# RobotLocomotion/pytorch-dense-correspondence

Measured on AMD Instinct MI355X. Metric: training images/sec, 640x480 D=3 ResNet34-8s, higher is better.
Workload: dtype f32 (f16x3 products)

## Files before the change

include/dcn_hip.h:

```cpp
#ifndef DCN_HIP_H
#define DCN_HIP_H

#include <stddef.h>
#include <stdint.h>

#ifdef __cplusplus
extern "C" {
#endif

#define DCN_OK 0
#define DCN_E_INVALID (-1)
#define DCN_E_LAUNCH (-2)
#define DCN_E_UNSUPPORTED (-3)

const char* dcn_version(void);

void dcn_reload_env(void);

void dcn_release_pooled_buffers(void);


enum { DCN_LIST_MATCH = 0, DCN_LIST_MASKED = 1, DCN_LIST_BACKGROUND = 2, DCN_LIST_BLIND = 3, DCN_NUM_LISTS = 4 };

enum {
// ... 76 lines not shown
int dcn_plan_bn_info(const dcn_plan* plan, int j, char* name, int name_cap, int64_t* channels);

int dcn_plan_fused_bn_backward(const dcn_plan* plan);

int dcn_plan_num_activation_slots(const dcn_plan* plan);
size_t dcn_plan_activation_absmax_offset(const dcn_plan* plan);

int dcn_plan_num_grad_buckets(const dcn_plan* plan);
int dcn_plan_grad_bucket_first_param(const dcn_plan* plan, int k);
int dcn_plan_stream_wait_grad_bucket(dcn_plan* plan, int k, void* stream);

size_t dcn_plan_saved_bytes(const dcn_plan* plan);
size_t dcn_plan_workspace_bytes(const dcn_plan* plan);
double dcn_plan_forward_flops(const dcn_plan* plan);

int dcn_backbone_forward(dcn_plan* plan, const float* image, const float* const* params,
                         float* const* bn_running, float momentum, float eps, int training, int normalize,
                         float* descriptors, void* saved, void* workspace, void* stream);

int dcn_backbone_forward_pair(dcn_plan* plan, const float* image_a, const float* image_b, const float* const* params,
                              float* const* bn_running, float momentum, float eps, int training, int normalize,
                              float* descriptors, void* saved, void* workspace, void* stream);

int dcn_plan_profile_begin(dcn_plan* plan);
int dcn_plan_profile_end(dcn_plan* plan, double ms[2], int64_t launches[2], double flops[2]);
int dcn_plan_profile_end3(dcn_plan* plan, double ms[3], int64_t launches[3], double flops[3]);
enum {
    DCN_PROF_GEMM = 0,
    DCN_PROF_WGRAD = 1,
    DCN_PROF_GEMM_HL = 2,
    DCN_PROF_BN_APPLY = 3,
    DCN_PROF_BN_BWD_REDUCE = 4,
    DCN_PROF_BN_BWD_APPLY = 5,
    DCN_PROF_BN_FINALIZE = 6,
    DCN_PROF_RESAMPLE = 7,
    DCN_PROF_OTHER = 8,
    DCN_PROF_NCAT = 9
};
int dcn_plan_profile_end_all(dcn_plan* plan, double ms[DCN_PROF_NCAT], int64_t launches[DCN_PROF_NCAT],
                             double work[DCN_PROF_NCAT]);

int dcn_backbone_backward(dcn_plan* plan, const float* grad_descriptors, const float* const* params,
                          const void* saved, void* workspace, float* const* grads, int normalize, void* stream);
int dcn_backbone_backward_pair(dcn_plan* plan, const float* grad_a, const float* grad_b, const float* const* params,
                               const void* saved, void* workspace, float* const* grads, int normalize, void* stream);


typedef struct dcn_conv_desc {
    int32_t n, hin, win, cin;
    int32_t hout, wout, cout;
    int32_t kh, kw, stride, pad, dil;
    int32_t ldc;
    int32_t group_rows;
} dcn_conv_desc;

int dcn_conv_forward(const dcn_conv_desc* c, const float* in, const float* w, const float* bias, float* out,
                     float* bn_partial, void* workspace, void* stream);
size_t dcn_conv_gemm_workspace(const dcn_conv_desc* c, int dgrad);
int dcn_conv_num_mtiles(const dcn_conv_desc* c);
int dcn_conv_dgrad(const dcn_conv_desc* c, const float* dout, const float* wt, const float* add, float* din,
                   void* workspace, void* stream);
int dcn_conv_wgrad(const dcn_conv_desc* c, const float* in, const float* dout, float* dw, void* slabs, void* stream);
size_t dcn_conv_wgrad_workspace(const dcn_conv_desc* c);
int dcn_transpose_weight(const float* w, float* wt, int cout, int taps, int cin, int ldn, void* stream);

int dcn_f16_kpad(int k);
int dcn_split_rows_f16(const float* w, void* hi, void* lo, int64_t rows, int k, float scale, void* stream);
int dcn_conv_num_mtiles_f16(const dcn_conv_desc* c);
size_t dcn_conv_gemm_workspace_f16(const dcn_conv_desc* c, int dgrad);
int dcn_conv_forward_f16(const dcn_conv_desc* c, const float* in, const float* in_absmax, const void* w_hi, const void* w_lo,
                         float w_scale, const float* bias, float* out, float* bn_partial, void* workspace, void* stream);
int dcn_conv_dgrad_f16(const dcn_conv_desc* c, const float* dout, const void* wt_hi, const void* wt_lo, float w_scale,
                       const float* dout_absmax, const float* add, float* din, void* workspace, void* stream);
int dcn_conv_dgrad_bn_num_mtiles_f16(const dcn_conv_desc* c);
int dcn_conv_dgrad_bn_f16(const dcn_conv_desc* c, const float* dout, const void* wt_hi, const void* wt_lo, float w_scale,
                          const float* dout_absmax, const float* add, float* din, const float* bn_x,
                          const unsigned char* relu_mask, const float* bn_stats, float* bn_partial, void* workspace,
                          void* stream);

int dcn_split_weights_checked_f16(int n, const float* const* w, const float* const* row_scale, void* const* hi, void* const* lo,
                                  const int* cout, const int* taps, const int* cin, float scale, int* status, void* stream);

int dcn_conv_hl_eligible(const dcn_conv_desc* c, int dgrad);
int dcn_conv_num_mtiles_hl(const dcn_conv_desc* c);
int dcn_conv_tile_rows_hl(const dcn_conv_desc* c, int dgrad);
size_t dcn_conv_gemm_workspace_hl(const dcn_conv_desc* c, int dgrad);
int dcn_conv_hl_shape_info(const dcn_conv_desc* c, int dgrad, int* info6);
int dcn_split_act_hl32(const float* src, const float* absmax, void* dst, int64_t rows, int channels, void* stream);
int dcn_split_weights_hl32(int n, const float* const* w, void* const* out, const int* cout, const int* taps, const int* cin,
                           const int* ldn, int transposed, float scale, void* stream);
int dcn_conv_forward_hl(const dcn_conv_desc* c, const void* in_hl, const float* in_absmax, const void* w_hl, float w_scale,
                        const float* bias, float* out, float* bn_partial, void* workspace, void* stream);
int dcn_conv_dgrad_hl(const dcn_conv_desc* c, const void* dout_hl, const void* wt_hl, float w_scale, const float* dout_absmax,
                      const float* add, float* din, void* workspace, void* stream);

int dcn_conv_wgrad_hl_eligible(const dcn_conv_desc* c);
int dcn_conv_wgrad_hl_kind(const dcn_conv_desc* c);
size_t dcn_conv_wgrad_workspace_hl(const dcn_conv_desc* c);
int dcn_conv_wgrad_hl(const dcn_conv_desc* c, const void* x_hl, const float* x_absmax, const void* dout_hl,
                      const float* dout_absmax, float* dw, void* slabs, void* stream);

int dcn_split_stem_weights_f16(const float* w4, void* hi, void* lo, int cout, float scale, void* stream);
int dcn_conv_stem_forward_f16(const dcn_conv_desc* c, const float* in, const float* in_absmax, const void* w_hi, const void* w_lo,
                              float w_scale, float* out, float* bn_partial, void* stream);

int dcn_split_weights_f16(int n, const float* const* w, void* const* hi, void* const* lo, const int* cout, const int* taps,
                          const int* cin, const int* ldn, int transposed, float scale, void* stream);

int dcn_split_weights_scaled_f16(int n, const float* const* w, const float* const* row_scale, void* const* hi,
                                 void* const* lo, const int* cout, const int* taps, const int* cin, const int* ldn,
                                 int transposed, float scale, void* stream);
int dcn_conv_forward_fused_f16(const dcn_conv_desc* c, const float* in, const float* in_absmax, const void* w_hi,
                               const void* w_lo, float w_scale, const float* bias, const float* add, int relu, float* out,
                               float* out_absmax, void* workspace, void* stream);

int dcn_split_act_f16(const float* src, void* xs, int64_t n, void* stream);
size_t dcn_grad_blocked_bytes(int m, int ld);
int dcn_split_grad_blocked_f16(const float* dy, int m, int ld, const float* absmax, void* dq, void* stream);
int dcn_conv_wgrad_f16(const dcn_conv_desc* c, const void* xs, int xs_is_fp32, const float* x_absmax, const void* dq,
                       const float* dout_absmax, float* dw, void* slabs, void* stream);
size_t dcn_conv_wgrad_workspace_f16(const dcn_conv_desc* c);

int dcn_bn_forward(const float* x, const float* bn_partial, int mtiles, int c, int64_t rows, const float* gamma,
                   const float* beta, float* running_mean, float* running_var, float momentum, float eps, int training,
                   const float* res, int relu, float* y, unsigned char* relu_mask, float* stats, void* stream);
size_t dcn_bn_backward_workspace(int64_t rows, int c);
int dcn_bn_backward(const float* dy, const unsigned char* relu_mask, const float* x, const float* stats, const float* gamma,
                    int c, int64_t rows, float* dgamma, float* dbeta, float* dx, float* g_out, void* workspace,
                    void* stream);
int dcn_bn_backward_from_partial(const float* dy, const float* bn_partial, int mtiles, const float* x, const float* stats,
                                 const float* gamma, int c, int64_t rows, float* dgamma, float* dbeta, float* dx,
                                 void* workspace, void* stream);
int dcn_maxpool_forward(const float* in, int n, int hin, int win, int c, float* out, unsigned char* argmax, void* stream);
int dcn_maxpool_backward(const float* gout, const unsigned char* argmax, int n, int hin, int win, int c, float* gin,
                         void* stream);

int dcn_upsample_forward(const float* low, int n, int hl, int wl, int ldl, int d, int h, int w, int normalize,
                         float* out, void* stream);
int dcn_upsample_backward(const float* gout, int n, int hl, int wl, int ldl, int d, int h, int w, float* glow,
                          float* tmp, void* stream);
size_t dcn_upsample_backward_tmp_bytes(int n, int hl, int w, int d);

size_t dcn_match_statistics_workspace(int q);
int dcn_match_statistics(const float* res, int64_t hw, int w, int d, const float* queries, const int64_t* gt_idx, int q,
                         const unsigned char* mask, int64_t* best_idx, float* best_dist, int32_t* count, float* dist_sum,
                         float* gt_dist, void* workspace, void* stream);

int dcn_find_best_match(const float* res, int64_t hw, int d, const float* queries, int q, const unsigned char* mask,
                        int64_t* best_idx, float* best_dist, float* norm_diffs, void* workspace, void* stream);
size_t dcn_find_best_match_workspace(int q);

size_t dcn_find_correspondences_workspace(int64_t n);
int dcn_find_correspondences(const uint16_t* depth_a, const uint16_t* depth_b, int h, int w, const float* K,
                             const float* K_inv, const float* pose_a, const float* pose_b_inv, const int64_t* cand_u,
                             const int64_t* cand_v, int64_t n, int64_t* out_ua, int64_t* out_va, float* out_ub,
                             float* out_vb, int64_t* out_count, void* workspace, void* stream);
size_t dcn_mask_nonzero_workspace(int64_t hw);
int dcn_mask_nonzero(const float* mask, int64_t hw, int64_t* list, int64_t* count, void* workspace, void* stream);
int dcn_sample_pixels(const float* rand, int64_t n, int w, int h, const int64_t* list, const int64_t* count, float* u,
                      float* v, void* stream);

int dcn_adam_step(int n, void* const* param, const void* const* grad, void* const* exp_avg, void* const* exp_avg_sq,
                  const int64_t* numel, double lr, double beta1, double beta2, double eps, double weight_decay,
                  int64_t step, void* stream);

#define DCN_AUG_PARAM_WORDS 16
// ... 103 lines not shown
```

pytorch-dense-correspondence_amd/csrc/conv_hl_kernels.hip:

```cpp
#include <algorithm>
#include <atomic>
#include <type_traits>

#include "conv_hlx.h"
#include "conv_shared.h"
#include "dcn_tuning.h"
#include "f16_split.h"

namespace {

using namespace dcnconv;
using namespace dcnsplit;

typedef __attribute__((address_space(3))) void* hl_lds_ptr;

constexpr int kOob = (int)0x80000000;
constexpr int kHlStage = 65536;
template <int MT> struct HlStage {
    static constexpr int kA = MT == 5 ? 320 * 128 : 32768, kStage = kA + 32768;
};
constexpr int HLK = 32;

__device__ __forceinline__ void glds16(__amdgpu_buffer_rsrc_t rs, void* lds_dst, int voffset, int soffset) {
    __builtin_amdgcn_raw_ptr_buffer_load_lds(rs, (hl_lds_ptr)lds_dst, 16, voffset, soffset, 0, 0);
}

__global__ void __launch_bounds__(256)
split_act_hl32_kernel(const float* __restrict__ src, const float* __restrict__ absmax, u32x4* __restrict__ dst, int64_t n8) {
    const float s = absmax ? pow2_scale(*absmax) : 1.f;
    for (int64_t i = (int64_t)blockIdx.x * 256 + threadIdx.x; i < n8; i += (int64_t)gridDim.x * 256) {
        const float4 a = reinterpret_cast<const float4*>(src)[2 * i], b = reinterpret_cast<const float4*>(src)[2 * i + 1];
        h4 ah, al, bh, bl;
        split4(a, s, ah, al);
        split4(b, s, bh, bl);
        const u32x2 h0 = __builtin_bit_cast(u32x2, ah), h1 = __builtin_bit_cast(u32x2, bh);
        const u32x2 l0 = __builtin_bit_cast(u32x2, al), l1 = __builtin_bit_cast(u32x2, bl);
        u32x4* line = dst + (i >> 2) * 8 + (i & 3);
        line[0] = u32x4{h0[0], h0[1], h1[0], h1[1]};
        line[4] = u32x4{l0[0], l0[1], l1[0], l1[1]};
    }
}

template <bool TR, int MT>
__device__ __forceinline__ void gemm_segment_hl(const GemmConv& p, unsigned char* lds, int tile, int k0, int k1, int nk,
                                                float* slot) {
    static_assert(MT == 3 || MT == 4 || MT == 5, "wavefront tiles of 96, 128 or 160 rows");
    constexpr int BM = 64 * MT, GR = 32 * MT;
    constexpr int NA = MT == 4 ? 4 : MT;
    constexpr int kHlStage = HlStage<MT>::kStage, kAB = HlStage<MT>::kA;
    const int tid = threadIdx.x, lane = tid & 63;
    const int wv = __builtin_amdgcn_readfirstlane(tid >> 6);
    const int grp = wv >> 2, wn = wv & 3;
    const int mt = fdiv(tile, p.div_nt), nt = tile - mt * p.ntiles;
    const int m0 = mt * BM, n0 = nt * 256;
    const __amdgpu_buffer_rsrc_t rs_a = __builtin_amdgcn_make_buffer_rsrc(const_cast<float*>(p.src), 0, (int)p.src_bytes, 0x00020000);
    const __amdgpu_buffer_rsrc_t rs_b = __builtin_amdgcn_make_buffer_rsrc(const_cast<_Float16*>(p.wh), 0, (int)p.w_bytes, 0x00020000);

    const int l8 = lane >> 3, ls = lane & 7;
    const int cs4 = p.cs * 4;
    auto a_piece_row = [&](int a) { return MT == 4 ? grp * 128 + (a >> 1) * 64 + (2 * wn + (a & 1)) * 8 : grp * GR + a * 32 + wn * 8; };
    int by[NA], bx[NA], rowoff[NA], voa[NA], vob[2][2];
    unsigned vmask[NA];
    int cur_delta = 0, cur_bit = 0;
#pragma unroll
    for (int a = 0; a < NA; ++a) {
        const int row = a_piece_row(a) + l8;
        const int sl = ls ^ ((row >> 1) & 7);
        const int m = m0 + row;
        const bool ok = m < p.M;
        const int mm = ok ? m : 0;
        const int img = fdiv(mm, p.div_hw), rem = mm - img * p.div_hw.d;
        const int y = fdiv(rem, p.div_w), x = rem - y * p.div_w.d;
        by[a] = ok ? (TR ? y + p.pad : y - p.pad) : -(1 << 28);
        bx[a] = TR ? x + p.pad : x - p.pad;
        rowoff[a] = ok ? (img * p.hs * p.ws + by[a] * p.ws + bx[a]) * cs4 + sl * 16 : 0;
        vmask[a] = 0u;
        if constexpr (MT == 5) {
            const int ntap = p.kh * p.kw;
            for (int tap = 0; tap < ntap; ++tap) {
                const int r = fdiv(tap, p.div_kw), s = tap - r * p.kw;
                const int dy = r * p.dil, dx = s * p.dil;
                bool v;
                if (TR) {
                    const int ny = by[a] - dy, nx = bx[a] - dx;
                    v = ((ny | nx) >= 0) & (ny < p.hs) & (nx < p.ws);
                } else {
// ... 464 lines not shown
    const HlxShape x = hlx_shape(M, cd, K, group_rows, taps, cs);
    const bool x_forced = force == 160 || tune.gemm_hlx_kg > 0 || tune.gemm_hlx_splits > 0;
    if (x.ok && (x_forced || !best.ok || x.cost < 0.97 * best_cost * best.nk)) {
        HlShape gx = best;
        gx.rows = kHlxRows; gx.mtiles = x.mtiles; gx.ntiles = x.ntiles; gx.nk = x.nk;
        gx.sk = false; gx.sk_wgs = 0; gx.sk_units = 0; gx.sk_dp = 0;
        gx.ws_bytes = x.ws_bytes; gx.sk_count_off = x.cnt_off;
        gx.ok = true;
        gx.x = x;
        return gx;
    }
    if (force == 160) best.ok = false;
    return best;
}

bool valid_desc_hl(const dcn_conv_desc* c) {
    return c && c->n > 0 && c->hin > 0 && c->win > 0 && c->cin > 0 && c->hout > 0 && c->wout > 0 && c->cout > 0 && c->kh > 0 &&
           c->kw > 0 && c->stride > 0 && c->dil > 0 && c->pad >= 0 && c->ldc >= c->cout;
}

template <int MT>
void launch_gemm_hl_rows(const GemmConv& p, bool sk, dim3 grid, hipStream_t st) {
    const dim3 block(512);
    if constexpr (MT != 5) {
        if (sk) {
            if (p.transposed) hipLaunchKernelGGL((conv_gemm_hl_kernel<true, true, MT>), grid, block, 0, st, p);
            else hipLaunchKernelGGL((conv_gemm_hl_kernel<false, true, MT>), grid, block, 0, st, p);
            return;
        }
    }
    {
        if (p.transposed) hipLaunchKernelGGL((conv_gemm_hl_kernel<true, false, MT>), grid, block, 0, st, p);
        else hipLaunchKernelGGL((conv_gemm_hl_kernel<false, false, MT>), grid, block, 0, st, p);
    }
}

int launch_gemm_hl(GemmConv& p, int group_rows, void* workspace, hipStream_t st) {
    if (p.relu || p.out_absmax || p.bnb_partial) return DCN_E_UNSUPPORTED;
    p.sshift = 0;
    p.div_hw = make_fastdiv(p.hd * p.wd);
    p.div_w = make_fastdiv(p.wd);
    p.div_cs = make_fastdiv(p.cs);
    p.div_kw = make_fastdiv(p.kw);
    const HlShape g = hl_shape(p.M, p.cd, p.K, group_rows, p.kh * p.kw, p.cs);
    if (!g.ok) return DCN_E_UNSUPPORTED;
    p.hl_setprio = dcn::tuning().hl_setprio;
    if (g.rows == kHlxRows) {
        if (g.x.splits > 1 && !workspace) {
            HlxShape x1 = g.x;
            x1.splits = 1; x1.ws_bytes = 0; x1.cnt_off = 0;
            return launch_gemm_hlx(p, x1, nullptr, st);
        }
        return launch_gemm_hlx(p, g.x, workspace, st);
    }
    const bool sk = g.sk && workspace != nullptr;
    p.mtiles = g.mtiles;
    p.ntiles = g.ntiles;
    p.div_nt = make_fastdiv(g.ntiles);
    p.div_nk = make_fastdiv(g.nk);
    p.sk_units = sk ? g.sk_units : 0;
    p.sk_dp = sk ? g.sk_dp : 0;
    p.sk_partial = sk ? (float*)workspace : nullptr;
    p.sk_count = sk ? (unsigned long long*)((char*)workspace + g.sk_count_off) : nullptr;
    p.sk_bytes = sk ? (unsigned)g.sk_count_off : 0u;
    if (sk) {
        p.sk_id = next_sk_launch_id();
        if (dcn::fill_bytes_async(p.sk_count, 0, (size_t)(g.mtiles * g.ntiles - g.sk_dp) * sizeof(unsigned long long), st) != DCN_OK)
            return DCN_E_LAUNCH;
    }
    const dim3 grid(sk ? g.sk_wgs : g.mtiles * g.ntiles);
    if (g.rows == 192) launch_gemm_hl_rows<3>(p, sk, grid, st);
    else if (g.rows == 320) launch_gemm_hl_rows<5>(p, false, grid, st);
    else launch_gemm_hl_rows<4>(p, sk, grid, st);
    return dcn::check_launch();
}

}

static HlShape hl_shape_of(const dcn_conv_desc* c, int dgrad) {
    if (dgrad) return hl_shape(c->n * c->hin * c->win, c->cin, c->kh * c->kw * c->ldc, 0, c->kh * c->kw, c->ldc);
    return hl_shape(c->n * c->hout * c->wout, c->cout, c->kh * c->kw * c->cin, c->group_rows, c->kh * c->kw, c->cin);
}

static bool hl_supported(const dcn_conv_desc* c, int dgrad) {
    if (!valid_desc_hl(c)) return false;
    if (c->stride != 1 || (c->ldc % 4) != 0) return false;
    const int cs = dgrad ? c->ldc : c->cin, cd = dgrad ? c->cin : c->cout;
    const int64_t M = (int64_t)c->n * (dgrad ? c->hin * c->win : c->hout * c->wout);
    const int64_t K = (int64_t)c->kh * c->kw * cs;
    if ((cs % HLK) != 0 || (dgrad && c->ldc != c->cout) || (cd % 4) != 0 || M >= ((int64_t)1 << 30)) return false;
    if (dgrad && (c->hin != c->hout || c->win != c->wout)) return false;
    const int64_t src_bytes = (int64_t)c->n * (dgrad ? c->hout * c->wout : c->hin * c->win) * cs * 4;
    const int64_t w_bytes = (int64_t)cd * K * 4;
    if (!(src_bytes <= ((int64_t)1 << 31) - 1 && w_bytes <= ((int64_t)1 << 31) - 1)) return false;
    return hl_shape_of(c, dgrad).ok;
}

extern "C" int dcn_conv_hl_eligible(const dcn_conv_desc* c, int dgrad) {
    if (!hl_supported(c, dgrad) || dcn::tuning().gemm_hl == 0) return 0;
    if (dcn::tuning().gemm_hl == 2) return 1;
    const int cs = dgrad ? c->ldc : c->cin, cd = dgrad ? c->cin : c->cout;
    const int64_t M = (int64_t)c->n * (dgrad ? c->hin * c->win : c->hout * c->wout);
    const int64_t K = (int64_t)c->kh * c->kw * cs;
    if (!(cd >= 128 && K >= std::min(512, dcn::tuning().hl_min_k) && M >= 4096)) return 0;
    const HlShape chosen = hl_shape_of(c, dgrad);
    if (chosen.rows == kHlxRows) return (cd >= 256 || cs >= 256 || dcn::tuning().gemm_hlx_narrow != 0) ? 1 : 0;
    if (cd < 256) return 0;
    if (chosen.rows == 320 && chosen.mtiles * chosen.ntiles <= 256 && chosen.mtiles * chosen.ntiles >= 120) return 1;
    const double rounds = (double)dcn::ceil_div64(M, 256) * dcn::ceil_div(cd, 256) / 256.0;
    if (rounds > 1.0 && rounds < 1.5 && K < 4096) return 0;
    if (rounds < 120.0 / 256.0) return 0;
    return 1;
}

extern "C" int dcn_conv_num_mtiles_hl(const dcn_conv_desc* c) {
    if (!valid_desc_hl(c)) return DCN_E_INVALID;
    return hl_shape_of(c, 0).mtiles;
}

extern "C" int dcn_conv_tile_rows_hl(const dcn_conv_desc* c, int dgrad) {
    if (!valid_desc_hl(c)) return DCN_E_INVALID;
    return hl_shape_of(c, dgrad).rows;
}

extern "C" size_t dcn_conv_gemm_workspace_hl(const dcn_conv_desc* c, int dgrad) {
    if (!valid_desc_hl(c)) return 0;
    return hl_shape_of(c, dgrad).ws_bytes;
}

extern "C" int dcn_conv_hl_shape_info(const dcn_conv_desc* c, int dgrad, int* info6) {
    if (!valid_desc_hl(c) || !info6) return DCN_E_INVALID;
    if (!hl_supported(c, dgrad)) return DCN_E_UNSUPPORTED;
    const HlShape g = hl_shape_of(c, dgrad);
    const bool x = g.rows == kHlxRows;
    info6[0] = g.rows; info6[1] = x ? g.x.bn : 256; info6[2] = x ? g.x.kg : 1; info6[3] = x ? g.x.splits : 1;
    info6[4] = g.mtiles; info6[5] = g.ntiles;
    return DCN_OK;
}

extern "C" int dcn_split_act_hl32(const float* src, const float* absmax, void* dst, int64_t rows, int channels, void* stream) {
    if (!src || !dst || rows < 1 || channels < HLK || (channels % HLK) != 0) return DCN_E_INVALID;
    const int64_t n8 = rows * (channels / 8);
    const unsigned blocks = (unsigned)(dcn::ceil_div64(n8, 256) > 8192 ? 8192 : dcn::ceil_div64(n8, 256));
    hipLaunchKernelGGL(split_act_hl32_kernel, dim3(blocks), dim3(256), 0, (hipStream_t)stream, src, absmax, (u32x4*)dst, n8);
    return dcn::check_launch();
}

extern "C" int dcn_conv_forward_hl(const dcn_conv_desc* c, const void* in_hl, const float* in_absmax, const void* w_hl,
                                   float w_scale, const float* bias, float* out, float* bn_partial, void* workspace,
                                   void* stream) {
    if (!in_hl || !w_hl || !out || !(w_scale > 0.f)) return DCN_E_INVALID;
    if (!hl_supported(c, 0)) return DCN_E_UNSUPPORTED;
    GemmConv p;
    p.src = (const float*)in_hl; p.wm = nullptr; p.bias = bias; p.add = nullptr; p.dst = out; p.bn_partial = bn_partial;
    p.out_absmax = nullptr; p.wh = (const _Float16*)w_hl; p.wl = nullptr; p.a_absmax = in_absmax; p.b_inv_scale = 1.f / w_scale;
    p.hs = c->hin; p.ws = c->win; p.cs = c->cin; p.hd = c->hout; p.wd = c->wout; p.cd = c->cout;
    p.kh = c->kh; p.kw = c->kw; p.stride = 1; p.pad = c->pad; p.dil = c->dil; p.ldc = c->ldc;
    p.M = c->n * c->hout * c->wout; p.K = c->kh * c->kw * c->cin; p.kp = p.K; p.transposed = 0; p.relu = 0;
    p.src_bytes = (unsigned)((int64_t)c->n * c->hin * c->win * c->cin * 4);
    p.w_bytes = (unsigned)((int64_t)c->cout * p.K * 4);
    return launch_gemm_hl(p, c->group_rows, workspace, (hipStream_t)stream);
}

extern "C" int dcn_conv_dgrad_hl(const dcn_conv_desc* c, const void* dout_hl, const void* wt_hl, float w_scale,
                                 const float* dout_absmax, const float* add, float* din, void* workspace, void* stream) {
    if (!dout_hl || !wt_hl || !din || !(w_scale > 0.f)) return DCN_E_INVALID;
    if (!hl_supported(c, 1)) return DCN_E_UNSUPPORTED;
    GemmConv p;
    p.src = (const float*)dout_hl; p.wm = nullptr; p.bias = nullptr; p.add = add; p.dst = din; p.bn_partial = nullptr;
    p.out_absmax = nullptr; p.wh = (const _Float16*)wt_hl; p.wl = nullptr; p.a_absmax = dout_absmax; p.b_inv_scale = 1.f / w_scale;
    p.hs = c->hout; p.ws = c->wout; p.cs = c->ldc; p.hd = c->hin; p.wd = c->win; p.cd = c->cin;
    p.kh = c->kh; p.kw = c->kw; p.stride = 1; p.pad = c->pad; p.dil = c->dil; p.ldc = c->cin;
    p.M = c->n * c->hin * c->win; p.K = c->kh * c->kw * c->ldc; p.kp = p.K; p.transposed = 1; p.relu = 0;
    p.src_bytes = (unsigned)((int64_t)c->n * c->hout * c->wout * c->ldc * 4);
    p.w_bytes = (unsigned)((int64_t)c->cin * p.K * 4);
    return launch_gemm_hl(p, 0, workspace, (hipStream_t)stream);
}
```

pytorch-dense-correspondence_amd/csrc/dcn_tuning.h:

```cpp
#pragma once

namespace dcn {

struct Tuning {
    int conv_mode = -1;
    int conv_mode_invalid = 0;
    int backward_overlap = 1;
    int gemm_tile_m = 0;
    int gemm_sk = -1;
    double gemm_sk_min_gain = 20.0;
    int gemm_uni = 1;
    int stem8 = 1;
    int gemm_sk_inline = 1;
    int bn_bwd_fused = 0;
    int defer_residual_add = 1;
    int wgrad_splits = 0;
    int wgrad_tile = 0;
    int wgrad_deep = 4;
    int gemm_hl = 1;
    int hl_min_k = 128;
    int gemm_hl_rows = 0;
    int gemm_hlx = 1;
    int gemm_hlx_kg = 0;
    int gemm_hlx_splits = 0;
    int gemm_hlx_narrow = 1;
    double hlx_cost1 = 1.32, hlx_cost2 = 1.42, hlx_split_cost = 14.0;
    int hl_setprio = 1;
    int hlx_stagger = 1;
    int hlx_counters = 1;
    int wgrad_hl_min_m = 0;
    int wgrad_hl = 1;
    int wgrad_hlr = 1;
    int wgrad_hlr_min_m = 0;
    int wgrad_hlr_pairs = 1;
    int hl_producers = 1;
    int hl_only_mid = 1;
    int stem_pool_fused = 1;
    int bn_reduce_wide = 32;
    int wsplit_overlap = 1;
    int bn_nt = 0;
    int bn_reverse = 0;
    int wgrad_roles = 1;
};

const Tuning& tuning();

}
```

pytorch-dense-correspondence_amd/csrc/dcn_tuning.hip:

```cpp
#include <atomic>
#include <cstdio>
#include <cstdlib>
#include <cstring>
#include <mutex>

#include "dcn_common.h"
#include "dcn_tuning.h"

namespace dcn {
namespace {

Tuning g_tuning;
std::once_flag g_once;
std::mutex g_mu;

void read_env(Tuning& t) {
    t = Tuning();
    if (const char* m = getenv("DCN_CONV_MODE")) {
        if (!strcmp(m, "fp32")) t.conv_mode = DCN_CONV_FP32;
        else if (!strcmp(m, "f16x3")) t.conv_mode = DCN_CONV_F16X3;
        else t.conv_mode_invalid = 1;
    }
    if (const char* e = getenv("DCN_BACKWARD_OVERLAP")) t.backward_overlap = atoi(e) != 0;
    if (const char* e = getenv("DCN_GEMM_TILE_M")) t.gemm_tile_m = atoi(e);
    if (const char* e = getenv("DCN_GEMM_SK")) t.gemm_sk = atoi(e);
    if (const char* e = getenv("DCN_GEMM_SK_MIN_GAIN")) t.gemm_sk_min_gain = atof(e);
    if (const char* e = getenv("DCN_STEM8")) t.stem8 = atoi(e) != 0;
    if (const char* e = getenv("DCN_GEMM_UNI")) t.gemm_uni = atoi(e) != 0;
    if (const char* e = getenv("DCN_GEMM_SK_FIXUP")) t.gemm_sk_inline = strcmp(e, "kernel") != 0;
    if (const char* e = getenv("DCN_BN_BWD_FUSED")) t.bn_bwd_fused = atoi(e) != 0;
    if (const char* e = getenv("DCN_DEFER_RESIDUAL_ADD")) t.defer_residual_add = atoi(e) != 0;
    if (const char* e = getenv("DCN_WGRAD_DEEP")) t.wgrad_deep = atoi(e);
    if (const char* e = getenv("DCN_WGRAD_ROLES")) t.wgrad_roles = atoi(e);
    if (const char* e = getenv("DCN_WGRAD_TILE")) t.wgrad_tile = atoi(e);
    if (const char* e = getenv("DCN_WGRAD_SPLITS")) t.wgrad_splits = atoi(e);
    if (const char* e = getenv("DCN_GEMM_HL")) t.gemm_hl = atoi(e);
    if (const char* e = getenv("DCN_GEMM_HL_ROWS")) t.gemm_hl_rows = atoi(e);
    if (const char* e = getenv("DCN_HL_MIN_K")) { const int v = atoi(e); if (v >= 32) t.hl_min_k = v; }
    if (const char* e = getenv("DCN_GEMM_HLX")) {
        int a = 0, b = 0;
        if (strchr(e, ',')) {
            if (sscanf(e, "%d,%d", &a, &b) == 2) {
                t.gemm_hlx = 1;
                t.gemm_hlx_kg = (a == 1 || a == 2) ? a : 0;
                t.gemm_hlx_splits = b > 0 ? b : 0;
            }
        } else {
            t.gemm_hlx = atoi(e) != 0;
        }
    }
    if (const char* e = getenv("DCN_GEMM_HLX_NARROW")) t.gemm_hlx_narrow = atoi(e) != 0;
    if (const char* e = getenv("DCN_HLX_COST")) {
        double a = 0, b = 0, c = 0;
        if (sscanf(e, "%lf,%lf,%lf", &a, &b, &c) == 3 && a > 0 && b > 0 && c >= 0) { t.hlx_cost1 = a; t.hlx_cost2 = b; t.hlx_split_cost = c; }
    }
    if (const char* e = getenv("DCN_HL_ONLY_MID")) t.hl_only_mid = atoi(e);
    if (const char* e = getenv("DCN_STEM_POOL_FUSED")) t.stem_pool_fused = atoi(e);
    if (const char* e = getenv("DCN_WGRAD_HL")) t.wgrad_hl = atoi(e);
    if (const char* e = getenv("DCN_HL_SETPRIO")) t.hl_setprio = atoi(e) != 0;
    if (const char* e = getenv("DCN_HLX_STAGGER")) { const int v = atoi(e); t.hlx_stagger = (v >= 0 && v <= 2) ? v : 1; }
    if (const char* e = getenv("DCN_HLX_COUNTERS")) t.hlx_counters = atoi(e) != 0;
    if (const char* e = getenv("DCN_WGRAD_HL_MIN_M")) t.wgrad_hl_min_m = atoi(e);
    if (const char* e = getenv("DCN_WGRAD_HLR")) t.wgrad_hlr = atoi(e);
    if (const char* e = getenv("DCN_WGRAD_HLR_MIN_M")) t.wgrad_hlr_min_m = atoi(e);
    if (const char* e = getenv("DCN_WGRAD_HLR_PAIRS")) t.wgrad_hlr_pairs = atoi(e);
    if (const char* e = getenv("DCN_HL_PRODUCERS")) t.hl_producers = atoi(e) != 0;
    if (const char* e = getenv("DCN_BN_REVERSE")) t.bn_reverse = atoi(e);
    if (const char* e = getenv("DCN_BN_NT")) t.bn_nt = atoi(e);
    if (const char* e = getenv("DCN_WSPLIT_OVERLAP")) t.wsplit_overlap = atoi(e) != 0;
    if (const char* e = getenv("DCN_BN_REDUCE_WIDE")) t.bn_reduce_wide = atoi(e);
}

}

const Tuning& tuning() {
    std::call_once(g_once, [] { read_env(g_tuning); });
    return g_tuning;
}

}

extern "C" void dcn_reload_env(void) {
    (void)dcn::tuning();
    std::lock_guard<std::mutex> lock(dcn::g_mu);
    dcn::read_env(dcn::g_tuning);
}
```

pytorch-dense-correspondence_amd/dcn_hip/_lib.py:

```python
import atexit
import ctypes
import os

import torch

HERE = os.path.dirname(os.path.abspath(__file__))
DEFAULT_PATH = os.path.join(HERE, "libdcn_hip.so")

_lib = None
_info = {"path": None, "version": None, "hostemu": False}
_reset_hooks = []

c_void_p, c_int, c_int64, c_size_t, c_float, c_char_p = (ctypes.c_void_p, ctypes.c_int, ctypes.c_int64,
                                                         ctypes.c_size_t, ctypes.c_float, ctypes.c_char_p)


class LossConfig(ctypes.Structure):
    _fields_ = [("margin", c_float * 4), ("invert", ctypes.c_int32 * 4), ("pixel_weight", ctypes.c_int32 * 4),
                ("m_pixel", c_float), ("image_width", ctypes.c_int32), ("match_loss_weight", c_float),
                ("non_match_loss_weight", c_float), ("scale_by_hard_negatives", ctypes.c_int32),
                ("compose", ctypes.c_int32)]


class ConvDesc(ctypes.Structure):
# ... 60 lines not shown
    "dcn_plan_profile_end3": (c_int, [c_void_p, ctypes.POINTER(ctypes.c_double), ctypes.POINTER(c_int64),
                                      ctypes.POINTER(ctypes.c_double)]),
    "dcn_plan_profile_end_all": (c_int, [c_void_p, ctypes.POINTER(ctypes.c_double), ctypes.POINTER(c_int64),
                                         ctypes.POINTER(ctypes.c_double)]),
    "dcn_backbone_forward": (c_int, [c_void_p, c_void_p, c_void_p, c_void_p, c_float, c_float, c_int, c_int, c_void_p,
                                     c_void_p, c_void_p, c_void_p]),
    "dcn_backbone_backward": (c_int, [c_void_p, c_void_p, c_void_p, c_void_p, c_void_p, c_void_p, c_int, c_void_p]),
    "dcn_backbone_forward_pair": (c_int, [c_void_p, c_void_p, c_void_p, c_void_p, c_void_p, c_float, c_float, c_int, c_int,
                                          c_void_p, c_void_p, c_void_p, c_void_p]),
    "dcn_backbone_backward_pair": (c_int, [c_void_p, c_void_p, c_void_p, c_void_p, c_void_p, c_void_p, c_void_p, c_int,
                                           c_void_p]),
    "dcn_conv_forward": (c_int, [ctypes.POINTER(ConvDesc), c_void_p, c_void_p, c_void_p, c_void_p, c_void_p, c_void_p,
                                 c_void_p]),
    "dcn_conv_gemm_workspace": (c_size_t, [ctypes.POINTER(ConvDesc), c_int]),
    "dcn_conv_num_mtiles": (c_int, [ctypes.POINTER(ConvDesc)]),
    "dcn_conv_dgrad": (c_int, [ctypes.POINTER(ConvDesc), c_void_p, c_void_p, c_void_p, c_void_p, c_void_p, c_void_p]),
    "dcn_conv_wgrad": (c_int, [ctypes.POINTER(ConvDesc), c_void_p, c_void_p, c_void_p, c_void_p, c_void_p]),
    "dcn_conv_wgrad_workspace": (c_size_t, [ctypes.POINTER(ConvDesc)]),
    "dcn_transpose_weight": (c_int, [c_void_p, c_void_p, c_int, c_int, c_int, c_int, c_void_p]),
    "dcn_f16_kpad": (c_int, [c_int]),
    "dcn_split_rows_f16": (c_int, [c_void_p, c_void_p, c_void_p, c_int64, c_int, c_float, c_void_p]),
    "dcn_conv_num_mtiles_f16": (c_int, [ctypes.POINTER(ConvDesc)]),
    "dcn_conv_gemm_workspace_f16": (c_size_t, [ctypes.POINTER(ConvDesc), c_int]),
    "dcn_conv_forward_f16": (c_int, [ctypes.POINTER(ConvDesc), c_void_p, c_void_p, c_void_p, c_void_p, c_float, c_void_p,
                                     c_void_p, c_void_p, c_void_p, c_void_p]),
    "dcn_conv_dgrad_f16": (c_int, [ctypes.POINTER(ConvDesc), c_void_p, c_void_p, c_void_p, c_float, c_void_p, c_void_p,
                                   c_void_p, c_void_p, c_void_p]),
    "dcn_split_stem_weights_f16": (c_int, [c_void_p, c_void_p, c_void_p, c_int, c_float, c_void_p]),
    "dcn_conv_stem_forward_f16": (c_int, [ctypes.POINTER(ConvDesc), c_void_p, c_void_p, c_void_p, c_void_p, c_float, c_void_p,
                                          c_void_p, c_void_p]),
    "dcn_conv_dgrad_bn_num_mtiles_f16": (c_int, [ctypes.POINTER(ConvDesc)]),
    "dcn_conv_dgrad_bn_f16": (c_int, [ctypes.POINTER(ConvDesc), c_void_p, c_void_p, c_void_p, c_float, c_void_p, c_void_p,
                                      c_void_p, c_void_p, c_void_p, c_void_p, c_void_p, c_void_p, c_void_p]),
    "dcn_bn_backward_from_partial": (c_int, [c_void_p, c_void_p, c_int, c_void_p, c_void_p, c_void_p, c_int, c_int64,
                                             c_void_p, c_void_p, c_void_p, c_void_p, c_void_p]),
    "dcn_triplet_loss_workspace_bytes": (c_size_t, [c_int64]),
    "dcn_triplet_loss_forward": (c_int, [c_void_p, c_void_p, c_int64, c_int, c_void_p, c_void_p, c_void_p, c_int64, c_int64,
                                         c_float, c_void_p, c_void_p, c_void_p, c_void_p]),
    "dcn_triplet_loss_backward": (c_int, [c_void_p, c_void_p, c_int64, c_int, c_void_p, c_void_p, c_void_p, c_int64, c_int64,
                                          c_float, c_void_p, c_void_p, c_void_p, c_void_p]),
    "dcn_find_correspondences_workspace": (c_size_t, [c_int64]),
    "dcn_find_correspondences": (c_int, [c_void_p, c_void_p, c_int, c_int, c_void_p, c_void_p, c_void_p, c_void_p, c_void_p,
                                         c_void_p, c_int64, c_void_p, c_void_p, c_void_p, c_void_p, c_void_p, c_void_p,
                                         c_void_p]),
    "dcn_mask_nonzero_workspace": (c_size_t, [c_int64]),
    "dcn_mask_nonzero": (c_int, [c_void_p, c_int64, c_void_p, c_void_p, c_void_p, c_void_p]),
    "dcn_sample_pixels": (c_int, [c_void_p, c_int64, c_int, c_int, c_void_p, c_void_p, c_void_p, c_void_p, c_void_p]),
    "dcn_adam_step": (c_int, [c_int, c_void_p, c_void_p, c_void_p, c_void_p, c_void_p, ctypes.c_double, ctypes.c_double,
                              ctypes.c_double, ctypes.c_double, ctypes.c_double, c_int64, c_void_p]),
    "dcn_plan_create_grouped": (c_int, [c_char_p, c_int, c_int, c_int, c_int, c_int, c_int, ctypes.POINTER(c_void_p)]),
    "dcn_plan_set_conv_mode": (c_int, [c_void_p, c_int]),
    "dcn_plan_conv_mode": (c_int, [c_void_p]),
    "dcn_conv_wgrad_f16": (c_int, [ctypes.POINTER(ConvDesc), c_void_p, c_int, c_void_p, c_void_p, c_void_p, c_void_p, c_void_p,
                                   c_void_p]),
    "dcn_split_weights_f16": (c_int, [c_int, c_void_p, c_void_p, c_void_p, c_void_p, c_void_p, c_void_p, c_void_p, c_int,
                                      c_float, c_void_p]),
    "dcn_split_weights_scaled_f16": (c_int, [c_int, c_void_p, c_void_p, c_void_p, c_void_p, c_void_p, c_void_p, c_void_p,
                                             c_void_p, c_int, c_float, c_void_p]),
    "dcn_conv_forward_fused_f16": (c_int, [ctypes.POINTER(ConvDesc), c_void_p, c_void_p, c_void_p, c_void_p, c_float, c_void_p,
                                           c_void_p, c_int, c_void_p, c_void_p, c_void_p, c_void_p]),
    "dcn_split_act_f16": (c_int, [c_void_p, c_void_p, c_int64, c_void_p]),
    "dcn_grad_blocked_bytes": (c_size_t, [c_int, c_int]),
    "dcn_split_grad_blocked_f16": (c_int, [c_void_p, c_int, c_int, c_void_p, c_void_p, c_void_p]),
    "dcn_conv_wgrad_workspace_f16": (c_size_t, [ctypes.POINTER(ConvDesc)]),
    "dcn_match_statistics_workspace": (c_size_t, [c_int]),
    "dcn_match_statistics": (c_int, [c_void_p, c_int64, c_int, c_int, c_void_p, c_void_p, c_int, c_void_p, c_void_p, c_void_p,
                                     c_void_p, c_void_p, c_void_p, c_void_p, c_void_p]),
    "dcn_find_best_match": (c_int, [c_void_p, c_int64, c_int, c_void_p, c_int, c_void_p, c_void_p, c_void_p, c_void_p,
                                    c_void_p, c_void_p]),
    "dcn_find_best_match_workspace": (c_size_t, [c_int]),
    "dcn_upsample_forward": (c_int, [c_void_p, c_int, c_int, c_int, c_int, c_int, c_int, c_int, c_int, c_void_p,
                                     c_void_p]),
    "dcn_upsample_backward": (c_int, [c_void_p, c_int, c_int, c_int, c_int, c_int, c_int, c_int, c_void_p, c_void_p,
                                      c_void_p]),
    "dcn_upsample_backward_tmp_bytes": (c_size_t, [c_int, c_int, c_int, c_int]),
    "dcn_split_weights_checked_f16": (c_int, [c_int, c_void_p, c_void_p, c_void_p, c_void_p, c_void_p, c_void_p, c_void_p,
                                              c_float, c_void_p, c_void_p]),
    "dcn_conv_wgrad_hl_eligible": (c_int, [ctypes.POINTER(ConvDesc)]),
    "dcn_conv_wgrad_hl_kind": (c_int, [ctypes.POINTER(ConvDesc)]),
    "dcn_conv_wgrad_workspace_hl": (c_size_t, [ctypes.POINTER(ConvDesc)]),
    "dcn_conv_wgrad_hl": (c_int, [ctypes.POINTER(ConvDesc), c_void_p, c_void_p, c_void_p, c_void_p, c_void_p, c_void_p, c_void_p]),
    "dcn_conv_hl_eligible": (c_int, [ctypes.POINTER(ConvDesc), c_int]),
    "dcn_conv_num_mtiles_hl": (c_int, [ctypes.POINTER(ConvDesc)]),
    "dcn_conv_tile_rows_hl": (c_int, [ctypes.POINTER(ConvDesc), c_int]),
    "dcn_conv_gemm_workspace_hl": (c_size_t, [ctypes.POINTER(ConvDesc), c_int]),
    "dcn_conv_hl_shape_info": (c_int, [ctypes.POINTER(ConvDesc), c_int, ctypes.POINTER(c_int)]),
    "dcn_split_act_hl32": (c_int, [c_void_p, c_void_p, c_void_p, c_int64, c_int, c_void_p]),
    "dcn_split_weights_hl32": (c_int, [c_int, c_void_p, c_void_p, c_void_p, c_void_p, c_void_p, c_void_p, c_int, c_float,
                                       c_void_p]),
    "dcn_conv_forward_hl": (c_int, [ctypes.POINTER(ConvDesc), c_void_p, c_void_p, c_void_p, c_float, c_void_p, c_void_p,
                                    c_void_p, c_void_p, c_void_p]),
    "dcn_conv_dgrad_hl": (c_int, [ctypes.POINTER(ConvDesc), c_void_p, c_void_p, c_float, c_void_p, c_void_p, c_void_p,
                                  c_void_p, c_void_p]),
    "dcn_augment_images": (c_int, [c_int, c_int, c_int, c_void_p, c_void_p, c_void_p, c_void_p, c_void_p, c_void_p, c_void_p,
                                   c_void_p, c_void_p, c_void_p, c_void_p, c_void_p, c_void_p, c_void_p, c_void_p]),
    "dcn_flip_planes": (c_int, [c_void_p, c_void_p, c_int64, c_int, c_int, c_int, c_int, c_int, c_void_p]),
    "dcn_flip_uv": (c_int, [c_int, c_void_p, c_void_p, c_void_p, c_void_p, c_int64, c_int, c_void_p, c_void_p, c_int, c_int,
                            c_int, c_void_p]),
    "dcn_merge_images": (c_int, [c_int, c_int, c_int, c_int] + [c_void_p] * 18),
    "dcn_merge_prune_workspace": (c_size_t, [c_int, c_int64, c_int64]),
    "dcn_sample_workspace": (c_size_t, [c_int, c_int, c_int, c_int64, c_int64]),
    "dcn_within_scene_samples": (c_int, [c_int, c_int, c_int] + [c_void_p] * 5 + [c_int64, c_int, c_int, c_int]
                                 + [c_void_p] * 4 + [c_int, c_void_p, c_void_p, c_int64] + [c_void_p] * 6),
    "dcn_complete_samples": (c_int, [c_int, c_int, c_int] + [c_void_p] * 4 + [c_int, c_void_p, c_int64, c_void_p, c_void_p,
                                                                              c_int, c_int, c_int] + [c_void_p] * 4
                             + [c_int, c_void_p, c_void_p, c_int64] + [c_void_p] * 6),
    "dcn_across_scene_samples": (c_int, [c_int, c_int, c_int, c_void_p, c_void_p, c_int64] + [c_void_p] * 4
                                 + [c_int, c_void_p, c_void_p, c_int64] + [c_void_p] * 6),
    "dcn_merge_prune": (c_int, [c_int, c_int, c_int] + [c_void_p] * 10 + [c_int64] + [c_void_p] * 5 + [c_int64, c_int]
                        + [c_void_p] * 9),
    "dcn_select_frames": (c_int, [c_int, c_int, ctypes.POINTER(FrameStoreDesc), c_int, ctypes.c_double, ctypes.c_double]
                          + [c_void_p] * 8),
    "dcn_gather_frames": (c_int, [c_int, c_int, ctypes.POINTER(FrameStoreDesc)] + [c_void_p] * 8),
}

ERRORS = {-1: "DCN_E_INVALID (bad argument)", -2: "DCN_E_LAUNCH (kernel launch failed)",
          -3: "DCN_E_UNSUPPORTED"}


def load(path=None):
    global _lib
    if _lib is not None and (path is None or os.path.abspath(path) == _info["path"]):
        return _lib
    p = os.path.abspath(path or os.environ.get("DCN_HIP_LIBRARY", DEFAULT_PATH))
    if not os.path.exists(p):
        raise RuntimeError(
            "dcn_hip: %s not found.  Build the gfx950 kernels first: `python __graft_entry__.py` "
            "(or dcn_hip.build.build_library()).  There is no CPU / PyTorch fallback for this path." % p)
    lib = ctypes.CDLL(p)
    for name, (res, args) in SYMBOLS.items():
        fn = getattr(lib, name)
        fn.restype = res
        fn.argtypes = args
    ver = lib.dcn_version().decode()
    for hook in _reset_hooks:
        hook()
    atexit.register(lib.dcn_release_pooled_buffers)
    _lib = lib
    _info.update(path=p, version=ver, hostemu=("hostemu" in ver))
    return _lib


def get():
    return _lib if _lib is not None else load()


def library_info():
    get()
    return dict(_info)


def is_hostemu():
    get()
    return _info["hostemu"]


def check(rc, what):
    if rc != 0:
        raise RuntimeError("dcn_hip: %s failed: %s" % (what, ERRORS.get(rc, rc)))


def require_device(*tensors):
    emu = is_hostemu()
    for t in tensors:
        if t is None:
            continue
# ... 16 lines not shown
```

Before: 456.9.

## Add windowed direct-conv kernel for 64-channel 3x3 stride-1 convolutions

Adds a specialized HL kernel for 3x3, stride-1, 64-in/64-out convolutions, used for both forward and dgrad. It keeps all nine taps' weights in registers and stages a 3-row pixel window in LDS with double-buffered async loads, so each input row is reused across taps instead of going through the generic im2col-style GEMM tiling. Eligibility and shape queries route these layers to the new kernel by default, which also bypasses the earlier minimum-size heuristics that may have rejected 64-channel layers. The kernel fuses the bias, the residual add and the BN partial statistics into its epilogue, and declines shapes that need relu or other outputs. The risk is lower occupancy (one 512-thread block per CU with large LDS) and correctness on edge tiles.

Result: no change. 457.3 (median of 5 runs) (+0.1%).

```diff
diff --git a/include/dcn_hip.h b/include/dcn_hip.h
--- a/include/dcn_hip.h
+++ b/include/dcn_hip.h
@@ -182,6 +182,7 @@
                                   const int* cout, const int* taps, const int* cin, float scale, int* status, void* stream);
 
 int dcn_conv_hl_eligible(const dcn_conv_desc* c, int dgrad);
+int dcn_conv_hl_kind(const dcn_conv_desc* c, int dgrad);
 int dcn_conv_num_mtiles_hl(const dcn_conv_desc* c);
 int dcn_conv_tile_rows_hl(const dcn_conv_desc* c, int dgrad);
 size_t dcn_conv_gemm_workspace_hl(const dcn_conv_desc* c, int dgrad);
diff --git a/pytorch-dense-correspondence_amd/csrc/conv_hl_kernels.hip b/pytorch-dense-correspondence_amd/csrc/conv_hl_kernels.hip
--- a/pytorch-dense-correspondence_amd/csrc/conv_hl_kernels.hip
+++ b/pytorch-dense-correspondence_amd/csrc/conv_hl_kernels.hip
@@ -2,6 +2,7 @@
 #include <atomic>
 #include <type_traits>
 
+#include "conv_hlw.h"
 #include "conv_hlx.h"
 #include "conv_shared.h"
 #include "dcn_tuning.h"
@@ -632,6 +633,13 @@
     return hl_shape(c->n * c->hout * c->wout, c->cout, c->kh * c->kw * c->cin, c->group_rows, c->kh * c->kw, c->cin);
 }
 
+static bool hlw_takes(const dcn_conv_desc* c, int dgrad) {
+    const dcn::Tuning& tune = dcn::tuning();
+    if (tune.gemm_hlw == 0 || tune.gemm_hl == 0 || !valid_desc_hl(c)) return false;
+    if (dgrad) return c->ldc == c->cout && hlw_supported(c->hout, c->wout, c->hin, c->win, c->ldc, c->cin, c->kh, c->kw, c->stride, c->pad, c->dil, 0);
+    return hlw_supported(c->hin, c->win, c->hout, c->wout, c->cin, c->cout, c->kh, c->kw, c->stride, c->pad, c->dil, c->group_rows);
+}
+
 static bool hl_supported(const dcn_conv_desc* c, int dgrad) {
     if (!valid_desc_hl(c)) return false;
     if (c->stride != 1 || (c->ldc % 4) != 0) return false;
@@ -643,12 +651,14 @@
     const int64_t src_bytes = (int64_t)c->n * (dgrad ? c->hout * c->wout : c->hin * c->win) * cs * 4;
     const int64_t w_bytes = (int64_t)cd * K * 4;
     if (!(src_bytes <= ((int64_t)1 << 31) - 1 && w_bytes <= ((int64_t)1 << 31) - 1)) return false;
+    if (hlw_takes(c, dgrad)) return true;
     return hl_shape_of(c, dgrad).ok;
 }
 
 extern "C" int dcn_conv_hl_eligible(const dcn_conv_desc* c, int dgrad) {
     if (!hl_supported(c, dgrad) || dcn::tuning().gemm_hl == 0) return 0;
     if (dcn::tuning().gemm_hl == 2) return 1;
+    if (hlw_takes(c, dgrad)) return 1;
     const int cs = dgrad ? c->ldc : c->cin, cd = dgrad ? c->cin : c->cout;
     const int64_t M = (int64_t)c->n * (dgrad ? c->hin * c->win : c->hout * c->wout);
     const int64_t K = (int64_t)c->kh * c->kw * cs;
@@ -665,22 +675,29 @@
 
 extern "C" int dcn_conv_num_mtiles_hl(const dcn_conv_desc* c) {
     if (!valid_desc_hl(c)) return DCN_E_INVALID;
+    if (hlw_takes(c, 0)) return hlw_tiles(c->n, c->hout, c->wout);
     return hl_shape_of(c, 0).mtiles;
 }
 
 extern "C" int dcn_conv_tile_rows_hl(const dcn_conv_desc* c, int dgrad) {
     if (!valid_desc_hl(c)) return DCN_E_INVALID;
+    if (hlw_takes(c, dgrad)) return kHlwPixels;
     return hl_shape_of(c, dgrad).rows;
 }
 
 extern "C" size_t dcn_conv_gemm_workspace_hl(const dcn_conv_desc* c, int dgrad) {
-    if (!valid_desc_hl(c)) return 0;
+    if (!valid_desc_hl(c) || hlw_takes(c, dgrad)) return 0;
     return hl_shape_of(c, dgrad).ws_bytes;
 }
 
 extern "C" int dcn_conv_hl_shape_info(const dcn_conv_desc* c, int dgrad, int* info6) {
     if (!valid_desc_hl(c) || !info6) return DCN_E_INVALID;
     if (!hl_supported(c, dgrad)) return DCN_E_UNSUPPORTED;
+    if (hlw_takes(c, dgrad)) {
+        info6[0] = kHlwPixels; info6[1] = 64; info6[2] = 1; info6[3] = 1;
+        info6[4] = hlw_tiles(c->n, dgrad ? c->hin : c->hout, dgrad ? c->win : c->wout); info6[5] = 1;
+        return DCN_OK;
+    }
     const HlShape g = hl_shape_of(c, dgrad);
     const bool x = g.rows == kHlxRows;
     info6[0] = g.rows; info6[1] = x ? g.x.bn : 256; info6[2] = x ? g.x.kg : 1; info6[3] = x ? g.x.splits : 1;
@@ -709,6 +726,7 @@
     p.M = c->n * c->hout * c->wout; p.K = c->kh * c->kw * c->cin; p.kp = p.K; p.transposed = 0; p.relu = 0;
     p.src_bytes = (unsigned)((int64_t)c->n * c->hin * c->win * c->cin * 4);
     p.w_bytes = (unsigned)((int64_t)c->cout * p.K * 4);
+    if (hlw_takes(c, 0)) return launch_gemm_hlw(p, c->n, (hipStream_t)stream);
     return launch_gemm_hl(p, c->group_rows, workspace, (hipStream_t)stream);
 }
 
@@ -724,5 +742,12 @@
     p.M = c->n * c->hin * c->win; p.K = c->kh * c->kw * c->ldc; p.kp = p.K; p.transposed = 1; p.relu = 0;
     p.src_bytes = (unsigned)((int64_t)c->n * c->hout * c->wout * c->ldc * 4);
     p.w_bytes = (unsigned)((int64_t)c->cin * p.K * 4);
+    if (hlw_takes(c, 1)) return launch_gemm_hlw(p, c->n, (hipStream_t)stream);
     return launch_gemm_hl(p, 0, workspace, (hipStream_t)stream);
 }
+
+extern "C" int dcn_conv_hl_kind(const dcn_conv_desc* c, int dgrad) {
+    if (!hl_supported(c, dgrad)) return 0;
+    if (hlw_takes(c, dgrad)) return 3;
+    return hl_shape_of(c, dgrad).rows == kHlxRows ? 2 : 1;
+}
diff --git a/pytorch-dense-correspondence_amd/csrc/conv_hlw.h b/pytorch-dense-correspondence_amd/csrc/conv_hlw.h
--- /dev/null
+++ b/pytorch-dense-correspondence_amd/csrc/conv_hlw.h
@@ -0,0 +1,12 @@
+#pragma once
+#include "conv_shared.h"
+
+namespace dcnconv {
+
+constexpr int kHlwPixels = 80;
+
+bool hlw_supported(int hs, int ws, int hd, int wd, int cs, int cd, int kh, int kw, int stride, int pad, int dil, int group_rows);
+int hlw_tiles(int n, int hd, int wd);
+int launch_gemm_hlw(GemmConv& p, int n, hipStream_t st);
+
+}
diff --git a/pytorch-dense-correspondence_amd/csrc/conv_hlw_kernels.hip b/pytorch-dense-correspondence_amd/csrc/conv_hlw_kernels.hip
--- /dev/null
+++ b/pytorch-dense-correspondence_amd/csrc/conv_hlw_kernels.hip
@@ -0,0 +1,193 @@
+#include <algorithm>
+
+#include "conv_hlw.h"
+#include "dcn_tuning.h"
+#include "f16_split.h"
+
+namespace {
+
+using namespace dcnconv;
+using namespace dcnsplit;
+
+typedef __attribute__((address_space(3))) void* hlw_lds_ptr;
+typedef f32x4_t f32x4;
+
+constexpr int kOob = (int)0x80000000;
+constexpr int WP = kHlwPixels;
+constexpr int WB = WP / 16;
+constexpr int WPITCH = 84;
+constexpr int kPix = 256;
+constexpr int kPieces = 3 * WPITCH / 4;
+constexpr int kWin = 3 * WPITCH * kPix;
+constexpr int KS = 18;
+constexpr int kRed = 4 * WB * 64 * 16;
+static_assert(WP % 16 == 0 && WPITCH >= WP + 2 && (3 * WPITCH) % 4 == 0, "window geometry");
+
+__device__ __forceinline__ void glds16w(__amdgpu_buffer_rsrc_t rs, void* lds_dst, int voffset) {
+    __builtin_amdgcn_raw_ptr_buffer_load_lds(rs, (hlw_lds_ptr)lds_dst, 16, voffset, 0, 0, 0);
+}
+
+template <bool TR>
+__global__ void __launch_bounds__(512, 1)
+conv_gemm_hlw_kernel(GemmConv p) {
+    __shared__ __attribute__((aligned(16))) unsigned char lds[2 * kWin + kRed];
+    const int tid = threadIdx.x, lane = tid & 63;
+    const int wv = __builtin_amdgcn_readfirstlane(tid >> 6);
+    const int cg = wv & 3, kg = wv >> 2;
+    const int fc = lane & 15, fq = lane >> 4;
+    const __amdgpu_buffer_rsrc_t rs_a = __builtin_amdgcn_make_buffer_rsrc(const_cast<float*>(p.src), 0, (int)p.src_bytes, 0x00020000);
+
+    h8 wb[9][2];
+    {
+        const unsigned char* wrow = reinterpret_cast<const unsigned char*>(p.wh) + (size_t)(cg * 16 + fc) * (KS * 128) + kg * 128 + fq * 16;
+#pragma unroll
+        for (int tap = 0; tap < 9; ++tap) {
+            wb[tap][0] = *reinterpret_cast<const h8*>(wrow + tap * 256);
+            wb[tap][1] = *reinterpret_cast<const h8*>(wrow + tap * 256 + 64);
+        }
+    }
+    const float sa = p.a_absmax ? pow2_scale(*p.a_absmax) : 1.f;
+    const float inv = p.b_inv_scale / sa;
+    const int segs = p.div_tiles.d, hd = p.div_hw.d;
+    const float bv = p.bias ? p.bias[cg * 16 + fc] : 0.f;
+    f32x4* red = reinterpret_cast<f32x4*>(lds + 2 * kWin) + cg * (WB * 64) + lane;
+
+    struct Org { int img, y, x; };
+    auto origin = [&](int t) {
+        const int row = fdiv(t, p.div_tiles), seg = t - row * segs;
+        const int img = fdiv(row, p.div_hw);
+        return Org{img, row - img * hd - 1, seg * WP - 1};
+    };
+    auto issue_piece = [&](const Org& o, unsigned char* win, int i) {
+        const int pc = wv + 8 * i;
+        if (pc < kPieces) {
+            const int wp = pc * 4 + (lane >> 4);
+            const int wr = wp / WPITCH, wx = wp - wr * WPITCH;
+            const int yy = o.y + wr, xx = o.x + wx;
+            const int q = (lane & 15) ^ ((wx & 7) << 1);
+            const bool ok = ((unsigned)yy < (unsigned)p.hs) & ((unsigned)xx < (unsigned)p.ws);
+            glds16w(rs_a, win + pc * 1024, ok ? ((o.img * p.hs + yy) * p.ws + xx) * kPix + q * 16 : kOob);
+        }
+    };
+    constexpr int kPiecesPerWave = (kPieces + 7) / 8;
+    static_assert(kPiecesPerWave <= 9, "one piece per tap");
+
+    int t = xcd_remap(blockIdx.x, gridDim.x);
+    if (t < p.mtiles) {
+        const Org o = origin(t);
+        for (int i = 0; i < kPiecesPerWave; ++i) issue_piece(o, lds, i);
+    }
+    int buf = 0;
+    for (; t < p.mtiles; t += gridDim.x, buf ^= 1) {
+        DCN_WAIT_VMCNT(0);
+        __syncthreads();
+        const bool more = t + (int)gridDim.x < p.mtiles;
+        const Org on = origin(more ? t + (int)gridDim.x : t);
+        unsigned char* wnext = lds + (buf ^ 1) * kWin;
+        const unsigned char* win = lds + buf * kWin;
+        int lc = fc;
+        DCN_OPAQUE_INT(lc);
+        f32x4 acc[WB];
+#pragma unroll
+        for (int b = 0; b < WB; ++b) acc[b] = f32x4{0.f, 0.f, 0.f, 0.f};
+        h8 fa[2][2][WB];
+        auto read = [&](int tap, int set) {
+            const int r = tap / 3, s = tap % 3;
+            const int wr = TR ? 2 - r : r, dx = TR ? 2 - s : s;
+#pragma unroll
+            for (int b = 0; b < WB; ++b) {
+                const int px = b * 16 + lc + dx;
+                const unsigned char* pix = win + (wr * WPITCH + px) * kPix;
+                const int sw = (px & 7) << 1;
+#pragma unroll
+                for (int pl = 0; pl < 2; ++pl)
+                    fa[set][pl][b] = *reinterpret_cast<const h8*>(pix + ((kg * 8 + pl * 4 + fq) ^ sw) * 16);
+            }
+        };
+        read(0, 0);
+#pragma unroll
+        for (int tap = 0; tap < 9; ++tap) {
+            const int set = tap & 1;
+            if (tap + 1 < 9) read(tap + 1, set ^ 1);
+            if (tap < kPiecesPerWave && more) issue_piece(on, wnext, tap);
+#pragma unroll
+            for (int b = 0; b < WB; ++b) acc[b] = __builtin_amdgcn_mfma_f32_16x16x32_f16(fa[set][1][b], wb[tap][0], acc[b], 0, 0, 0);
+#pragma unroll
+            for (int b = 0; b < WB; ++b) acc[b] = __builtin_amdgcn_mfma_f32_16x16x32_f16(fa[set][0][b], wb[tap][1], acc[b], 0, 0, 0);
+#pragma unroll
+            for (int b = 0; b < WB; ++b) acc[b] = __builtin_amdgcn_mfma_f32_16x16x32_f16(fa[set][0][b], wb[tap][0], acc[b], 0, 0, 0);
+            __builtin_amdgcn_sched_barrier(0);
+        }
+        if (kg == 1) {
+#pragma unroll
+            for (int b = 0; b < WB; ++b) red[b * 64] = acc[b];
+        }
+        __syncthreads();
+        if (kg == 1) continue;
+#pragma unroll
+        for (int b = 0; b < WB; ++b) acc[b] += red[b * 64];
+
+        const int row = fdiv(t, p.div_tiles), seg = t - row * segs;
+        const int x0 = seg * WP;
+        const int64_t m0 = (int64_t)row * p.wd + x0;
+        const int col = cg * 16 + lc;
+        float csum = 0.f, csq = 0.f, cmax = 0.f;
+#pragma unroll
+        for (int b = 0; b < WB; ++b) {
+#pragma unroll
+            for (int e = 0; e < 4; ++e) {
+                const int xo = b * 16 + 4 * fq + e;
+                if (x0 + xo < p.wd) {
+                    const float a = acc[b][e] * inv;
+                    const int64_t o = (m0 + xo) * p.ldc + col;
+                    float v = a + bv;
+                    if (p.add) v += p.add[o];
+                    p.dst[o] = v;
+                    csum += a;
+                    csq = fmaf(a, a, csq);
+                    cmax = fmaxf(cmax, fabsf(a));
+                }
+            }
+        }
+        if (p.bn_partial) {
+            csum += __shfl_xor(csum, 16, 64);
+            csq += __shfl_xor(csq, 16, 64);
+            cmax = fmaxf(cmax, __shfl_xor(cmax, 16, 64));
+            csum += __shfl_xor(csum, 32, 64);
+            csq += __shfl_xor(csq, 32, 64);
+            cmax = fmaxf(cmax, __shfl_xor(cmax, 32, 64));
+            if (fq == 0) {
+                p.bn_partial[((int64_t)t * 3 + 0) * p.cd + col] = csum;
+                p.bn_partial[((int64_t)t * 3 + 1) * p.cd + col] = csq;
+                p.bn_partial[((int64_t)t * 3 + 2) * p.cd + col] = cmax;
+            }
+        }
+    }
+}
+
+}
+
+namespace dcnconv {
+
+bool hlw_supported(int hs, int ws, int hd, int wd, int cs, int cd, int kh, int kw, int stride, int pad, int dil, int group_rows) {
+    if (kh != 3 || kw != 3 || stride != 1 || pad != 1 || dil != 1 || cs != 64 || cd != 64) return false;
+    if (hs != hd || ws != wd || hd < 1 || wd < 1) return false;
+    return group_rows <= 0 || (group_rows % (hd * wd)) == 0;
+}
+
+int hlw_tiles(int n, int hd, int wd) { return n * hd * dcn::ceil_div(wd, WP); }
+
+int launch_gemm_hlw(GemmConv& p, int n, hipStream_t st) {
+    if (p.relu || p.out_absmax || p.bnb_partial) return DCN_E_UNSUPPORTED;
+    const int tiles = hlw_tiles(n, p.hd, p.wd);
+    p.mtiles = tiles;
+    p.ntiles = 1;
+    p.div_tiles = make_fastdiv(dcn::ceil_div(p.wd, WP));
+    p.div_hw = make_fastdiv(p.hd);
+    const int grid = std::min(tiles, 256);
+    if (p.transposed) hipLaunchKernelGGL((conv_gemm_hlw_kernel<true>), dim3(grid), dim3(512), 0, st, p);
+    else hipLaunchKernelGGL((conv_gemm_hlw_kernel<false>), dim3(grid), dim3(512), 0, st, p);
+    return dcn::check_launch();
+}
+
+}
diff --git a/pytorch-dense-correspondence_amd/csrc/dcn_tuning.h b/pytorch-dense-correspondence_amd/csrc/dcn_tuning.h
--- a/pytorch-dense-correspondence_amd/csrc/dcn_tuning.h
+++ b/pytorch-dense-correspondence_amd/csrc/dcn_tuning.h
@@ -24,6 +24,7 @@
     int gemm_hlx_kg = 0;
     int gemm_hlx_splits = 0;
     int gemm_hlx_narrow = 1;
+    int gemm_hlw = 1;
     double hlx_cost1 = 1.32, hlx_cost2 = 1.42, hlx_split_cost = 14.0;
     int hl_setprio = 1;
     int hlx_stagger = 1;
diff --git a/pytorch-dense-correspondence_amd/csrc/dcn_tuning.hip b/pytorch-dense-correspondence_amd/csrc/dcn_tuning.hip
--- a/pytorch-dense-correspondence_amd/csrc/dcn_tuning.hip
+++ b/pytorch-dense-correspondence_amd/csrc/dcn_tuning.hip
@@ -50,6 +50,7 @@
         }
     }
     if (const char* e = getenv("DCN_GEMM_HLX_NARROW")) t.gemm_hlx_narrow = atoi(e) != 0;
+    if (const char* e = getenv("DCN_GEMM_HLW")) t.gemm_hlw = atoi(e);
     if (const char* e = getenv("DCN_HLX_COST")) {
         double a = 0, b = 0, c = 0;
         if (sscanf(e, "%lf,%lf,%lf", &a, &b, &c) == 3 && a > 0 && b > 0 && c >= 0) { t.hlx_cost1 = a; t.hlx_cost2 = b; t.hlx_split_cost = c; }
diff --git a/pytorch-dense-correspondence_amd/dcn_hip/_lib.py b/pytorch-dense-correspondence_amd/dcn_hip/_lib.py
--- a/pytorch-dense-correspondence_amd/dcn_hip/_lib.py
+++ b/pytorch-dense-correspondence_amd/dcn_hip/_lib.py
@@ -166,6 +166,7 @@
     "dcn_conv_wgrad_hl": (c_int, [ctypes.POINTER(ConvDesc), c_void_p, c_void_p, c_void_p, c_void_p, c_void_p, c_void_p, c_void_p]),
     "dcn_conv_hl_eligible": (c_int, [ctypes.POINTER(ConvDesc), c_int]),
     "dcn_conv_num_mtiles_hl": (c_int, [ctypes.POINTER(ConvDesc)]),
+    "dcn_conv_hl_kind": (c_int, [ctypes.POINTER(ConvDesc), c_int]),
     "dcn_conv_tile_rows_hl": (c_int, [ctypes.POINTER(ConvDesc), c_int]),
     "dcn_conv_gemm_workspace_hl": (c_size_t, [ctypes.POINTER(ConvDesc), c_int]),
     "dcn_conv_hl_shape_info": (c_int, [ctypes.POINTER(ConvDesc), c_int, ctypes.POINTER(c_int)]),
```
